# SamsungLabs/fcaf3d

Measured on AMD Instinct MI355X. Metric: scenes/sec fwd+bwd, ScanNet 100k-pt 2cm voxels, 1/2/4/8 MI355X, higher is better.
Workload: dtype f32

## Files before the change

fcaf3d_amd/csrc/norm_bn.h:

```cpp
#pragma once


__global__ void k_bn1_partial(const float* __restrict__ x, int64_t n, int C, int64_t rpb, float* __restrict__ part) {
  extern __shared__ float sm[];
  const auto [cl, rl, nrl] = lane_coord(C / 4);
  const auto [r0, r1] = row_span(rpb, n);
  const float4 sh = *reinterpret_cast<const float4*>(x + cl * 4);
  float4 a1 = make_float4(0.f, 0.f, 0.f, 0.f), a2 = a1;
  for (int64_t rb = r0 + rl; rb < r1; rb += 4 * (int64_t)nrl) {
    float4 v[4];
#pragma unroll
    for (int u = 0; u < 4; ++u) {
      const int64_t r = rb + (int64_t)u * nrl;
      v[u] = *reinterpret_cast<const float4*>(x + (r < r1 ? r : 0) * C + cl * 4);
    }
#pragma unroll
    for (int u = 0; u < 4; ++u) {
      v[u].x -= sh.x; v[u].y -= sh.y; v[u].z -= sh.z; v[u].w -= sh.w;
      a1.x += v[u].x; a1.y += v[u].y; a1.z += v[u].z; a1.w += v[u].w;
      a2.x += v[u].x * v[u].x; a2.y += v[u].y * v[u].y; a2.z += v[u].z * v[u].z; a2.w += v[u].w * v[u].w;
    }
  }
  *reinterpret_cast<float4*>(&sm[(rl * 2 + 0) * C + cl * 4]) = a1;
  *reinterpret_cast<float4*>(&sm[(rl * 2 + 1) * C + cl * 4]) = a2;
  __syncthreads();
  if (rl == 0) {
    float4 t1 = make_float4(0.f, 0.f, 0.f, 0.f), t2 = t1;
    for (int j = 0; j < nrl; ++j) {
      float4 u = *reinterpret_cast<const float4*>(&sm[(j * 2 + 0) * C + cl * 4]);
      float4 w = *reinterpret_cast<const float4*>(&sm[(j * 2 + 1) * C + cl * 4]);
      t1.x += u.x; t1.y += u.y; t1.z += u.z; t1.w += u.w;
      t2.x += w.x; t2.y += w.y; t2.z += w.z; t2.w += w.w;
    }
    float* dst = part + ((int64_t)blockIdx.x * 2) * C;
    *reinterpret_cast<float4*>(dst + cl * 4) = t1;
    *reinterpret_cast<float4*>(dst + C + cl * 4) = t2;
  }
}

__device__ static inline void bn1_reduce_parts(const float* __restrict__ part, int nb, int C, int cl, int rl, int nrl,
                                               float* sm , float4* s1, float4* s2, int CG, int c0) {
  float4 a1 = make_float4(0.f, 0.f, 0.f, 0.f), a2 = a1;
  const bool past_l1 = (int64_t)nb * C * 8 <= 32768;
  for (int b = rl; b < nb; b += nrl) {
    const float* src = part + ((int64_t)b * 2) * C + c0;
    float4 u = past_l1 ? fc_ld4(src + cl * 4) : *reinterpret_cast<const float4*>(src + cl * 4);
    float4 w = past_l1 ? fc_ld4(src + C + cl * 4) : *reinterpret_cast<const float4*>(src + C + cl * 4);
    a1.x += u.x; a1.y += u.y; a1.z += u.z; a1.w += u.w;
    a2.x += w.x; a2.y += w.y; a2.z += w.z; a2.w += w.w;
  }
  *reinterpret_cast<float4*>(&sm[(rl * 2 + 0) * CG + cl * 4]) = a1;
  *reinterpret_cast<float4*>(&sm[(rl * 2 + 1) * CG + cl * 4]) = a2;
  __syncthreads();
  float4 t1 = make_float4(0.f, 0.f, 0.f, 0.f), t2 = t1;
  for (int j = 0; j < nrl; ++j) {
    float4 u = *reinterpret_cast<const float4*>(&sm[(j * 2 + 0) * CG + cl * 4]);
    float4 w = *reinterpret_cast<const float4*>(&sm[(j * 2 + 1) * CG + cl * 4]);
    t1.x += u.x; t1.y += u.y; t1.z += u.z; t1.w += u.w;
    t2.x += w.x; t2.y += w.y; t2.z += w.z; t2.w += w.w;
  }
  *s1 = t1; *s2 = t2;
}

__global__ void k_bn1_apply(const float* __restrict__ x, int64_t n, int C, int64_t rpb, const float* __restrict__ part, int nb,
                            float eps, const float* __restrict__ gamma, const float* __restrict__ beta,
                            const float* __restrict__ residual, int act, float momentum, float* __restrict__ y,
                            float* __restrict__ mean_out, float* __restrict__ var_out, float* __restrict__ cnt_out,
                            float* __restrict__ rmean, float* __restrict__ rvar, long long* __restrict__ nbt,
                            const int* __restrict__ add_inv, const float* __restrict__ add_src) {
  extern __shared__ float sm[];
  const int c4n = C / 4;
  const int cl = threadIdx.x % c4n, rl = threadIdx.x / c4n;
  const int nrl = blockDim.x / c4n;
  float4 s1, s2;
  bn1_reduce_parts(part, nb, C, cl, rl, nrl, sm, &s1, &s2, C, 0);
  const float4 sh = *reinterpret_cast<const float4*>(x + cl * 4);
  const float inv_n = 1.f / (float)n;
  float d[4] = {s1.x * inv_n, s1.y * inv_n, s1.z * inv_n, s1.w * inv_n};
  float q[4] = {s2.x * inv_n, s2.y * inv_n, s2.z * inv_n, s2.w * inv_n};
  float shv[4] = {sh.x, sh.y, sh.z, sh.w};
  float mu[4], va[4], is[4], g[4], bt[4];
#pragma unroll
  for (int j = 0; j < 4; ++j) {
    mu[j] = shv[j] + d[j];
    va[j] = fmaxf(q[j] - d[j] * d[j], 0.f);
    is[j] = 1.f / sqrtf(va[j] + eps);
    g[j] = gamma ? gamma[cl * 4 + j] : 1.f;
    bt[j] = beta ? beta[cl * 4 + j] : 0.f;
  }
  if (blockIdx.x == 0 && rl == 0) {
    *reinterpret_cast<float4*>(mean_out + cl * 4) = make_float4(mu[0], mu[1], mu[2], mu[3]);
    *reinterpret_cast<float4*>(var_out + cl * 4) = make_float4(va[0], va[1], va[2], va[3]);
    if (cl == 0) { cnt_out[0] = (float)n; if (nbt) nbt[0] += 1; }
    if (rmean) {
#pragma unroll
      for (int j = 0; j < 4; ++j) bn_running_update(rmean, rvar, cl * 4 + j, mu[j], va[j], (float)n, momentum);
    }
  }
  const auto [r0, r1] = row_span(rpb, n);
  for (int64_t rb = r0 + rl; rb < r1; rb += 4 * (int64_t)nrl) {
    float v[4][4], rs[4][4];
#pragma unroll
    for (int u = 0; u < 4; ++u) {
      const int64_t r = rb + (int64_t)u * nrl;
      const int64_t rc = r < r1 ? r : r0;
      *reinterpret_cast<float4*>(v[u]) = *reinterpret_cast<const float4*>(x + rc * C + cl * 4);
      if (residual) *reinterpret_cast<float4*>(rs[u]) = *reinterpret_cast<const float4*>(residual + rc * C + cl * 4);
    }
#pragma unroll
    for (int u = 0; u < 4; ++u) {
      const int64_t r = rb + (int64_t)u * nrl;
      if (r >= r1) continue;
      float o[4];
#pragma unroll
      for (int j = 0; j < 4; ++j) o[j] = norm_act_elem(v[u][j], mu[j], is[j], g[j], bt[j], residual ? &rs[u][j] : nullptr, act);
      const int q = add_inv ? add_inv[r] : -1;
      if (q >= 0) {
        const float4 f = *reinterpret_cast<const float4*>(add_src + (int64_t)q * C + cl * 4);
        o[0] += f.x; o[1] += f.y; o[2] += f.z; o[3] += f.w;
      }
      *reinterpret_cast<float4*>(y + r * C + cl * 4) = *reinterpret_cast<float4*>(o);
    }
  }
}

__global__ __launch_bounds__(1024) void k_bn_finalize(const float* __restrict__ part, int nb, int C, int64_t n,
                                                      const float* __restrict__ x, float momentum, float* __restrict__ mean,
                                                      float* __restrict__ var, float* __restrict__ cnt,
                                                      float* __restrict__ rmean, float* __restrict__ rvar,
                                                      long long* __restrict__ nbt) {
  __shared__ float r1[16][65], r2[16][65];
  const int c = blockIdx.x * 64 + (threadIdx.x & 63), j = threadIdx.x >> 6;
  float a1 = 0.f, a2 = 0.f;
  if (c < C) {
    float p1[4] = {0.f, 0.f, 0.f, 0.f}, p2[4] = {0.f, 0.f, 0.f, 0.f};
    int b = j;
    for (; b + 48 < nb; b += 64) {
      float u[4], w[4];
#pragma unroll
      for (int q = 0; q < 4; ++q) {
        u[q] = fc_ld(&part[((int64_t)(b + 16 * q) * 2) * C + c]);
        w[q] = fc_ld(&part[((int64_t)(b + 16 * q) * 2 + 1) * C + c]);
      }
#pragma unroll
      for (int q = 0; q < 4; ++q) { p1[q] += u[q]; p2[q] += w[q]; }
    }
    for (; b < nb; b += 16) {
      p1[0] += fc_ld(&part[((int64_t)b * 2) * C + c]);
      p2[0] += fc_ld(&part[((int64_t)b * 2 + 1) * C + c]);
    }
    a1 = (p1[0] + p1[1]) + (p1[2] + p1[3]);
    a2 = (p2[0] + p2[1]) + (p2[2] + p2[3]);
  }
  r1[j][threadIdx.x & 63] = a1;
  r2[j][threadIdx.x & 63] = a2;
  __syncthreads();
  if (j == 0 && c < C) {
    float s1 = 0.f, s2 = 0.f;
    for (int q = 0; q < 16; ++q) { s1 += r1[q][threadIdx.x & 63]; s2 += r2[q][threadIdx.x & 63]; }
    const float inv_n = 1.f / (float)n;
    float d = s1 * inv_n;
    float mu = x[c] + d;
    float va = fmaxf(s2 * inv_n - d * d, 0.f);
    mean[c] = mu;
    var[c] = va;
    if (c == 0) { cnt[0] = (float)n; if (nbt) nbt[0] += 1; }
    if (rmean) bn_running_update(rmean, rvar, c, mu, va, (float)n, momentum);
  }
}

__global__ void k_bn1_bwd_apply(const float* __restrict__ x, const float* __restrict__ y, const float* __restrict__ gy,
                                const float* __restrict__ gy2, int64_t n, int C, int64_t rpb, const float* __restrict__ part, int nb,
                                const float* __restrict__ mean, const float* __restrict__ var, float eps,
                                const float* __restrict__ gamma, const float* __restrict__ beta, int act,
                                float* __restrict__ gx, float* __restrict__ gres, float* __restrict__ sums , int CG,
                                unsigned* __restrict__ amax_out) {
  extern __shared__ float sm[];
  const int c0 = blockIdx.y * CG;
  x += c0; gy += c0; gx += c0; mean += c0; var += c0;
  if (y) y += c0;
  if (gy2) gy2 += c0;
  if (gres) gres += c0;
  if (gamma) gamma += c0;
  if (beta) beta += c0;
  const int c4n = CG / 4;
  const int cl = threadIdx.x % c4n, rl = threadIdx.x / c4n;
  const int nrl = blockDim.x / c4n;
  float4 t1, t2;
  bn1_reduce_parts(part, nb, C, cl, rl, nrl, sm, &t1, &t2, CG, c0);
  if (blockIdx.x == 0 && rl == 0) {
    *reinterpret_cast<float4*>(sums + c0 + cl * 4) = t1;
    *reinterpret_cast<float4*>(sums + C + c0 + cl * 4) = t2;
  }
  const float inv_n = 1.f / (float)n;
  float s1[4] = {t1.x * inv_n, t1.y * inv_n, t1.z * inv_n, t1.w * inv_n};
  float s2[4] = {t2.x * inv_n, t2.y * inv_n, t2.z * inv_n, t2.w * inv_n};
  float mu[4], is[4], g[4], bt[4];
#pragma unroll
  for (int j = 0; j < 4; ++j) {
    mu[j] = mean[cl * 4 + j];
    is[j] = 1.f / sqrtf(var[cl * 4 + j] + eps);
    g[j] = gamma ? gamma[cl * 4 + j] : 1.f;
    bt[j] = beta ? beta[cl * 4 + j] : 0.f;
  }
  const bool from_y = act && y;
  const auto [r0, r1] = row_span(rpb, n);
  unsigned am = 0u;
  for (int64_t rb = r0 + rl; rb < r1; rb += 4 * (int64_t)nrl) {
    float xv[4][4], gv[4][4], yv[4][4];
#pragma unroll
    for (int u = 0; u < 4; ++u) {
      const int64_t r = rb + (int64_t)u * nrl;
      const int64_t rc = r < r1 ? r : r0;
      *reinterpret_cast<float4*>(xv[u]) = *reinterpret_cast<const float4*>(x + rc * C + cl * 4);
      *reinterpret_cast<float4*>(gv[u]) = *reinterpret_cast<const float4*>(gy + rc * C + cl * 4);
      if (gy2) {
        const float4 t2 = *reinterpret_cast<const float4*>(gy2 + rc * C + cl * 4);
        gv[u][0] += t2.x; gv[u][1] += t2.y; gv[u][2] += t2.z; gv[u][3] += t2.w;
      }
      if (from_y) *reinterpret_cast<float4*>(yv[u]) = *reinterpret_cast<const float4*>(y + rc * C + cl * 4);
    }
#pragma unroll
    for (int u = 0; u < 4; ++u) {
      const int64_t r = rb + (int64_t)u * nrl;
      if (r >= r1) continue;
      float o[4], gr[4];
#pragma unroll
      for (int j = 0; j < 4; ++j) {
        float gg = gv[u][j];
        if (from_y) gg *= act_bwd_from_y(yv[u][j], act);
        else if (act) gg *= act_bwd_from_pre(bn_pre(xv[u][j], mu[j], is[j], g[j], bt[j]), act);
        float xh = (xv[u][j] - mu[j]) * is[j];
        gr[j] = gg;
        o[j] = g[j] * is[j] * (gg - s1[j] - xh * s2[j]);
      }
      *reinterpret_cast<float4*>(gx + r * C + cl * 4) = *reinterpret_cast<float4*>(o);
      if (gres) *reinterpret_cast<float4*>(gres + r * C + cl * 4) = *reinterpret_cast<float4*>(gr);
#pragma unroll
      for (int j = 0; j < 4; ++j) amax_fold(am, o[j]);
    }
  }
  if (amax_out) amax_commit(am, amax_out);
}

__global__ void k_bn2_apply(const float* __restrict__ x, int64_t n, int C, int64_t rpb, const float* __restrict__ part, int nb, int G,
                            float eps, const float* __restrict__ gamma, const float* __restrict__ beta,
                            const float* __restrict__ residual, int act, float momentum, float* __restrict__ y,
                            float* __restrict__ mean_out, float* __restrict__ var_out, float* __restrict__ cnt_out,
                            float* __restrict__ rmean, float* __restrict__ rvar, long long* __restrict__ nbt, int CG,
                            const int* __restrict__ add_inv, const float* __restrict__ add_src, unsigned* __restrict__ amax_out) {
  extern __shared__ double smd[];
  const int c0 = blockIdx.y * CG;
  x += c0; y += c0; part += c0; mean_out += c0; var_out += c0;
  if (add_src) add_src += c0;
  if (residual) residual += c0;
  if (gamma) gamma += c0;
  if (beta) beta += c0;
  if (rmean) { rmean += c0; rvar += c0; }
  const auto [cl, rl, nrl] = lane_coord(CG / 4);
  double a1[4] = {0., 0., 0., 0.}, a2[4] = {0., 0., 0., 0.};
  const int GC = G * C;
  for (int t = rl; t < nb * G; t += nrl) {
    const int b = t / G, g = t % G;
    const float* src = part + ((int64_t)b * 2) * GC + g * C + cl * 4;
    const float4 u = fc_ld4(src), w = fc_ld4(src + GC);
    a1[0] += u.x; a1[1] += u.y; a1[2] += u.z; a1[3] += u.w;
    a2[0] += w.x; a2[1] += w.y; a2[2] += w.z; a2[3] += w.w;
  }
#pragma unroll
  for (int j = 0; j < 4; ++j) {
    smd[(rl * 2 + 0) * CG + cl * 4 + j] = a1[j];
    smd[(rl * 2 + 1) * CG + cl * 4 + j] = a2[j];
  }
  __syncthreads();
  float mu[4], va[4], is[4], g[4], bt[4];
#pragma unroll
  for (int j = 0; j < 4; ++j) {
    double t1 = 0., t2 = 0.;
    for (int q = 0; q < nrl; ++q) { t1 += smd[(q * 2 + 0) * CG + cl * 4 + j]; t2 += smd[(q * 2 + 1) * CG + cl * 4 + j]; }
    bn2_stats(t1, t2, n, &mu[j], &va[j]);
    is[j] = 1.f / sqrtf(va[j] + eps);
    g[j] = gamma ? gamma[cl * 4 + j] : 1.f;
    bt[j] = beta ? beta[cl * 4 + j] : 0.f;
  }
  if (blockIdx.x == 0 && rl == 0) {
    *reinterpret_cast<float4*>(mean_out + cl * 4) = make_float4(mu[0], mu[1], mu[2], mu[3]);
    *reinterpret_cast<float4*>(var_out + cl * 4) = make_float4(va[0], va[1], va[2], va[3]);
    if (cl == 0 && blockIdx.y == 0) { cnt_out[0] = (float)n; if (nbt) nbt[0] += 1; }
    if (rmean) {
#pragma unroll
      for (int j = 0; j < 4; ++j) bn_running_update(rmean, rvar, cl * 4 + j, mu[j], va[j], (float)n, momentum);
    }
  }
  const auto [r0, r1] = row_span(rpb, n);
  unsigned am = 0u;
  for (int64_t rb = r0 + rl; rb < r1; rb += 4 * (int64_t)nrl) {
    float v[4][4], rs[4][4];
    int q[4];
#pragma unroll
    for (int u = 0; u < 4; ++u) {
      const int64_t r = rb + (int64_t)u * nrl;
      const int64_t rc = r < r1 ? r : r0;
      *reinterpret_cast<float4*>(v[u]) = *reinterpret_cast<const float4*>(x + rc * C + cl * 4);
      if (residual) *reinterpret_cast<float4*>(rs[u]) = *reinterpret_cast<const float4*>(residual + rc * C + cl * 4);
      q[u] = add_inv ? add_inv[rc] : -1;
    }
#pragma unroll
    for (int u = 0; u < 4; ++u) {
      const int64_t r = rb + (int64_t)u * nrl;
      if (r >= r1) continue;
      float o[4];
#pragma unroll
      for (int j = 0; j < 4; ++j) o[j] = norm_act_elem(v[u][j], mu[j], is[j], g[j], bt[j], residual ? &rs[u][j] : nullptr, act);
      if (q[u] >= 0) {
        const float4 f = *reinterpret_cast<const float4*>(add_src + (int64_t)q[u] * C + cl * 4);
        o[0] += f.x; o[1] += f.y; o[2] += f.z; o[3] += f.w;
      }
      *reinterpret_cast<float4*>(y + r * C + cl * 4) = *reinterpret_cast<float4*>(o);
#pragma unroll
      for (int j = 0; j < 4; ++j) amax_fold(am, o[j]);
    }
  }
  if (amax_out) amax_commit(am, amax_out);
}

__global__ __launch_bounds__(256) void k_bn2_finalize(const float* __restrict__ part, int nb, int C, int G, int64_t n, float momentum,
                                                       float* __restrict__ mean, float* __restrict__ var, float* __restrict__ cnt,
                                                       float* __restrict__ rmean, float* __restrict__ rvar,
                                                       long long* __restrict__ nbt) {
  __shared__ double r1[FIN_SL][FIN_CB + 1], r2[FIN_SL][FIN_CB + 1];
  const int cl = threadIdx.x & (FIN_CB - 1), j = threadIdx.x / FIN_CB;
  const int c = blockIdx.x * FIN_CB + cl;
  const int GC = G * C;
  double a1 = 0., a2 = 0.;
  if (c < C) {
    double p1[4] = {0., 0., 0., 0.}, p2[4] = {0., 0., 0., 0.};
    const int total = nb * G;
    int t = j;
    for (; t + 3 * FIN_SL < total; t += 4 * FIN_SL) {
      float u[4], w[4];
#pragma unroll
      for (int q = 0; q < 4; ++q) {
        const int tt = t + FIN_SL * q, b = tt / G, g = tt % G;
        u[q] = fc_ld(&part[((int64_t)b * 2) * GC + g * C + c]);
        w[q] = fc_ld(&part[((int64_t)b * 2 + 1) * GC + g * C + c]);
      }
#pragma unroll
      for (int q = 0; q < 4; ++q) { p1[q] += u[q]; p2[q] += w[q]; }
    }
    for (; t < total; t += FIN_SL) {
      const int b = t / G, g = t % G;
      p1[0] += fc_ld(&part[((int64_t)b * 2) * GC + g * C + c]);
      p2[0] += fc_ld(&part[((int64_t)b * 2 + 1) * GC + g * C + c]);
    }
    a1 = (p1[0] + p1[1]) + (p1[2] + p1[3]);
    a2 = (p2[0] + p2[1]) + (p2[2] + p2[3]);
  }
  r1[j][cl] = a1;
  r2[j][cl] = a2;
  __syncthreads();
  if (j == 0 && c < C) {
    double s1 = 0., s2 = 0.;
    for (int q = 0; q < FIN_SL; ++q) { s1 += r1[q][cl]; s2 += r2[q][cl]; }
    float mu, va;
    bn2_stats(s1, s2, n, &mu, &va);
    mean[c] = mu;
    var[c] = va;
    if (c == 0) { cnt[0] = (float)n; if (nbt) nbt[0] += 1; }
    if (rmean) bn_running_update(rmean, rvar, c, mu, va, (float)n, momentum);
  }
}

extern "C" __global__ void k_bn_running(const float* __restrict__ mean, const float* __restrict__ var, const float* __restrict__ cnt,
                             float momentum, int C, float* __restrict__ rmean, float* __restrict__ rvar,
                             long long* __restrict__ nbt) {
  int c = blockIdx.x * blockDim.x + threadIdx.x;
  if (c == 0 && nbt) nbt[0] += 1;
  if (c >= C) return;
  float n = cnt[0];
  float unbias = n / fmaxf(n - 1.f, 1.f);
  rmean[c] = (1.f - momentum) * rmean[c] + momentum * mean[c];
  rvar[c] = (1.f - momentum) * rvar[c] + momentum * var[c] * unbias;
}
```

Before: 542.7.

## Overlap first row-tile loads with BN partial reduction and batch partial loads

In the BN backward apply and BN2 apply kernels, the first tile of activation rows is now loaded before the cross-block partial-sum reduction, so global-memory latency overlaps the reduction. The partial-sum reduction loops are unrolled by four with a scheduling barrier, putting several loads in flight at once. BN2 also prefetches gathered add_src rows and splits the per-channel stats across lanes with shuffles when CG is 64. 256-thread launch bounds are added. The cost is more live registers from the preloaded tiles, which may reduce occupancy.

```diff
diff --git a/fcaf3d_amd/csrc/norm_bn.h b/fcaf3d_amd/csrc/norm_bn.h
--- a/fcaf3d_amd/csrc/norm_bn.h
+++ b/fcaf3d_amd/csrc/norm_bn.h
@@ -38,16 +38,28 @@
   }
 }
 
+#define AP_TB 4
+
 __device__ static inline void bn1_reduce_parts(const float* __restrict__ part, int nb, int C, int cl, int rl, int nrl,
                                                float* sm , float4* s1, float4* s2, int CG, int c0) {
   float4 a1 = make_float4(0.f, 0.f, 0.f, 0.f), a2 = a1;
   const bool past_l1 = (int64_t)nb * C * 8 <= 32768;
-  for (int b = rl; b < nb; b += nrl) {
-    const float* src = part + ((int64_t)b * 2) * C + c0;
-    float4 u = past_l1 ? fc_ld4(src + cl * 4) : *reinterpret_cast<const float4*>(src + cl * 4);
-    float4 w = past_l1 ? fc_ld4(src + C + cl * 4) : *reinterpret_cast<const float4*>(src + C + cl * 4);
-    a1.x += u.x; a1.y += u.y; a1.z += u.z; a1.w += u.w;
-    a2.x += w.x; a2.y += w.y; a2.z += w.z; a2.w += w.w;
+  for (int b0 = rl; b0 < nb; b0 += AP_TB * nrl) {
+    float4 u[AP_TB], w[AP_TB];
+#pragma unroll
+    for (int q = 0; q < AP_TB; ++q) {
+      const int b = b0 + q * nrl;
+      const float* src = part + ((int64_t)(b < nb ? b : b0) * 2) * C + c0;
+      u[q] = past_l1 ? fc_ld4(src + cl * 4) : *reinterpret_cast<const float4*>(src + cl * 4);
+      w[q] = past_l1 ? fc_ld4(src + C + cl * 4) : *reinterpret_cast<const float4*>(src + C + cl * 4);
+    }
+    __builtin_amdgcn_sched_barrier(0);
+#pragma unroll
+    for (int q = 0; q < AP_TB; ++q) {
+      if (b0 + q * nrl >= nb) continue;
+      a1.x += u[q].x; a1.y += u[q].y; a1.z += u[q].z; a1.w += u[q].w;
+      a2.x += w[q].x; a2.y += w[q].y; a2.z += w[q].z; a2.w += w[q].w;
+    }
   }
   *reinterpret_cast<float4*>(&sm[(rl * 2 + 0) * CG + cl * 4]) = a1;
   *reinterpret_cast<float4*>(&sm[(rl * 2 + 1) * CG + cl * 4]) = a2;
@@ -169,7 +181,7 @@
   }
 }
 
-__global__ void k_bn1_bwd_apply(const float* __restrict__ x, const float* __restrict__ y, const float* __restrict__ gy,
+__global__ __launch_bounds__(256) void k_bn1_bwd_apply(const float* __restrict__ x, const float* __restrict__ y, const float* __restrict__ gy,
                                 const float* __restrict__ gy2, int64_t n, int C, int64_t rpb, const float* __restrict__ part, int nb,
                                 const float* __restrict__ mean, const float* __restrict__ var, float eps,
                                 const float* __restrict__ gamma, const float* __restrict__ beta, int act,
@@ -186,6 +198,31 @@
   const int c4n = CG / 4;
   const int cl = threadIdx.x % c4n, rl = threadIdx.x / c4n;
   const int nrl = blockDim.x / c4n;
+  const bool from_y = act && y;
+  const RowSpan span = row_span(rpb, n);
+  const int64_t r0 = span.r0, r1 = span.r1;
+  float xv[4][4], gv[4][4], g2[4][4], yv[4][4];
+  const auto load_rows = [&](int64_t rb) {
+#pragma unroll
+    for (int u = 0; u < 4; ++u) {
+      const int64_t r = rb + (int64_t)u * nrl;
+      const int64_t rc = r < r1 ? r : r0;
+      *reinterpret_cast<float4*>(xv[u]) = *reinterpret_cast<const float4*>(x + rc * C + cl * 4);
+      *reinterpret_cast<float4*>(gv[u]) = *reinterpret_cast<const float4*>(gy + rc * C + cl * 4);
+      if (gy2) *reinterpret_cast<float4*>(g2[u]) = *reinterpret_cast<const float4*>(gy2 + rc * C + cl * 4);
+      if (from_y) *reinterpret_cast<float4*>(yv[u]) = *reinterpret_cast<const float4*>(y + rc * C + cl * 4);
+    }
+  };
+  int64_t rb = r0 + rl;
+  if (rb < r1) load_rows(rb);
+  float mu[4], va[4], is[4], g[4], bt[4];
+#pragma unroll
+  for (int j = 0; j < 4; ++j) {
+    mu[j] = mean[cl * 4 + j];
+    va[j] = var[cl * 4 + j];
+    g[j] = gamma ? gamma[cl * 4 + j] : 1.f;
+    bt[j] = beta ? beta[cl * 4 + j] : 0.f;
+  }
   float4 t1, t2;
   bn1_reduce_parts(part, nb, C, cl, rl, nrl, sm, &t1, &t2, CG, c0);
   if (blockIdx.x == 0 && rl == 0) {
@@ -195,30 +232,14 @@
   const float inv_n = 1.f / (float)n;
   float s1[4] = {t1.x * inv_n, t1.y * inv_n, t1.z * inv_n, t1.w * inv_n};
   float s2[4] = {t2.x * inv_n, t2.y * inv_n, t2.z * inv_n, t2.w * inv_n};
-  float mu[4], is[4], g[4], bt[4];
-#pragma unroll
-  for (int j = 0; j < 4; ++j) {
-    mu[j] = mean[cl * 4 + j];
-    is[j] = 1.f / sqrtf(var[cl * 4 + j] + eps);
-    g[j] = gamma ? gamma[cl * 4 + j] : 1.f;
-    bt[j] = beta ? beta[cl * 4 + j] : 0.f;
-  }
-  const bool from_y = act && y;
-  const auto [r0, r1] = row_span(rpb, n);
+#pragma unroll
+  for (int j = 0; j < 4; ++j) is[j] = 1.f / sqrtf(va[j] + eps);
   unsigned am = 0u;
-  for (int64_t rb = r0 + rl; rb < r1; rb += 4 * (int64_t)nrl) {
-    float xv[4][4], gv[4][4], yv[4][4];
-#pragma unroll
-    for (int u = 0; u < 4; ++u) {
-      const int64_t r = rb + (int64_t)u * nrl;
-      const int64_t rc = r < r1 ? r : r0;
-      *reinterpret_cast<float4*>(xv[u]) = *reinterpret_cast<const float4*>(x + rc * C + cl * 4);
-      *reinterpret_cast<float4*>(gv[u]) = *reinterpret_cast<const float4*>(gy + rc * C + cl * 4);
-      if (gy2) {
-        const float4 t2 = *reinterpret_cast<const float4*>(gy2 + rc * C + cl * 4);
-        gv[u][0] += t2.x; gv[u][1] += t2.y; gv[u][2] += t2.z; gv[u][3] += t2.w;
-      }
-      if (from_y) *reinterpret_cast<float4*>(yv[u]) = *reinterpret_cast<const float4*>(y + rc * C + cl * 4);
+  for (bool first = true; rb < r1; rb += 4 * (int64_t)nrl, first = false) {
+    if (!first) load_rows(rb);
+    if (gy2) {
+#pragma unroll
+      for (int u = 0; u < 4; ++u) { gv[u][0] += g2[u][0]; gv[u][1] += g2[u][1]; gv[u][2] += g2[u][2]; gv[u][3] += g2[u][3]; }
     }
 #pragma unroll
     for (int u = 0; u < 4; ++u) {
@@ -243,7 +264,7 @@
   if (amax_out) amax_commit(am, amax_out);
 }
 
-__global__ void k_bn2_apply(const float* __restrict__ x, int64_t n, int C, int64_t rpb, const float* __restrict__ part, int nb, int G,
+__global__ __launch_bounds__(256) void k_bn2_apply(const float* __restrict__ x, int64_t n, int C, int64_t rpb, const float* __restrict__ part, int nb, int G,
                             float eps, const float* __restrict__ gamma, const float* __restrict__ beta,
                             const float* __restrict__ residual, int act, float momentum, float* __restrict__ y,
                             float* __restrict__ mean_out, float* __restrict__ var_out, float* __restrict__ cnt_out,
@@ -257,31 +278,90 @@
   if (gamma) gamma += c0;
   if (beta) beta += c0;
   if (rmean) { rmean += c0; rvar += c0; }
-  const auto [cl, rl, nrl] = lane_coord(CG / 4);
+  const LaneCoord lane = lane_coord(CG / 4);
+  const RowSpan span = row_span(rpb, n);
+  const int cl = lane.cl, rl = lane.rl, nrl = lane.nrl;
+  const int64_t r0 = span.r0, r1 = span.r1;
+  float v[4][4], rs[4][4];
+  int q[4];
+  const auto load_rows = [&](int64_t rb) {
+#pragma unroll
+    for (int u = 0; u < 4; ++u) {
+      const int64_t r = rb + (int64_t)u * nrl;
+      const int64_t rc = r < r1 ? r : r0;
+      *reinterpret_cast<float4*>(v[u]) = *reinterpret_cast<const float4*>(x + rc * C + cl * 4);
+      if (residual) *reinterpret_cast<float4*>(rs[u]) = *reinterpret_cast<const float4*>(residual + rc * C + cl * 4);
+      q[u] = add_inv ? add_inv[rc] : -1;
+    }
+  };
+  float4 f[4];
+  const auto load_adds = [&](int64_t rb) {
+#pragma unroll
+    for (int u = 0; u < 4; ++u)
+      if (rb + (int64_t)u * nrl < r1 && q[u] >= 0) f[u] = *reinterpret_cast<const float4*>(add_src + (int64_t)q[u] * C + cl * 4);
+  };
+  int64_t rb = r0 + rl;
+  if (rb < r1) load_rows(rb);
+  float mu[4], va[4], is[4], g[4], bt[4];
+#pragma unroll
+  for (int j = 0; j < 4; ++j) {
+    g[j] = gamma ? gamma[cl * 4 + j] : 1.f;
+    bt[j] = beta ? beta[cl * 4 + j] : 0.f;
+  }
   double a1[4] = {0., 0., 0., 0.}, a2[4] = {0., 0., 0., 0.};
-  const int GC = G * C;
-  for (int t = rl; t < nb * G; t += nrl) {
-    const int b = t / G, g = t % G;
-    const float* src = part + ((int64_t)b * 2) * GC + g * C + cl * 4;
-    const float4 u = fc_ld4(src), w = fc_ld4(src + GC);
-    a1[0] += u.x; a1[1] += u.y; a1[2] += u.z; a1[3] += u.w;
-    a2[0] += w.x; a2[1] += w.y; a2[2] += w.z; a2[3] += w.w;
-  }
+  const int GC = G * C, T = nb * G;
+  int t0 = rl;
+  do {
+    float4 u[AP_TB], w[AP_TB];
+#pragma unroll
+    for (int p = 0; p < AP_TB; ++p) {
+      const int t = t0 + p * nrl, tc = t < T ? t : T - 1;
+      const int b = tc / G, gi = tc % G;
+      const float* src = part + ((int64_t)b * 2) * GC + gi * C + cl * 4;
+      u[p] = fc_ld4(src), w[p] = fc_ld4(src + GC);
+    }
+    __builtin_amdgcn_sched_barrier(0);
+#pragma unroll
+    for (int p = 0; p < AP_TB; ++p) {
+      const bool in = t0 + p * nrl < T;
+      const float us[4] = {u[p].x, u[p].y, u[p].z, u[p].w}, ws[4] = {w[p].x, w[p].y, w[p].z, w[p].w};
+#pragma unroll
+      for (int j = 0; j < 4; ++j) {
+        const double n1 = a1[j] + us[j], n2 = a2[j] + ws[j];
+        a1[j] = in ? n1 : a1[j];
+        a2[j] = in ? n2 : a2[j];
+      }
+    }
+    t0 += AP_TB * nrl;
+  } while (t0 < T);
+  if (add_inv && rb < r1) load_adds(rb);
 #pragma unroll
   for (int j = 0; j < 4; ++j) {
     smd[(rl * 2 + 0) * CG + cl * 4 + j] = a1[j];
     smd[(rl * 2 + 1) * CG + cl * 4 + j] = a2[j];
   }
   __syncthreads();
-  float mu[4], va[4], is[4], g[4], bt[4];
-#pragma unroll
-  for (int j = 0; j < 4; ++j) {
+  if (CG == 64 && nrl == 16) {
+    const int j = rl & 3;
     double t1 = 0., t2 = 0.;
-    for (int q = 0; q < nrl; ++q) { t1 += smd[(q * 2 + 0) * CG + cl * 4 + j]; t2 += smd[(q * 2 + 1) * CG + cl * 4 + j]; }
-    bn2_stats(t1, t2, n, &mu[j], &va[j]);
-    is[j] = 1.f / sqrtf(va[j] + eps);
-    g[j] = gamma ? gamma[cl * 4 + j] : 1.f;
-    bt[j] = beta ? beta[cl * 4 + j] : 0.f;
+    for (int p = 0; p < 16; ++p) { t1 += smd[(p * 2 + 0) * CG + cl * 4 + j]; t2 += smd[(p * 2 + 1) * CG + cl * 4 + j]; }
+    float m, v;
+    bn2_stats(t1, t2, n, &m, &v);
+    const float s = 1.f / sqrtf(v + eps);
+#pragma unroll
+    for (int k = 0; k < 4; ++k) {
+      mu[k] = __shfl(m, k * 16 + cl);
+      va[k] = __shfl(v, k * 16 + cl);
+      is[k] = __shfl(s, k * 16 + cl);
+    }
+  } else {
+#pragma unroll
+    for (int j = 0; j < 4; ++j) {
+      double t1 = 0., t2 = 0.;
+      for (int p = 0; p < nrl; ++p) { t1 += smd[(p * 2 + 0) * CG + cl * 4 + j]; t2 += smd[(p * 2 + 1) * CG + cl * 4 + j]; }
+      bn2_stats(t1, t2, n, &mu[j], &va[j]);
+      is[j] = 1.f / sqrtf(va[j] + eps);
+    }
   }
   if (blockIdx.x == 0 && rl == 0) {
     *reinterpret_cast<float4*>(mean_out + cl * 4) = make_float4(mu[0], mu[1], mu[2], mu[3]);
@@ -292,18 +372,11 @@
       for (int j = 0; j < 4; ++j) bn_running_update(rmean, rvar, cl * 4 + j, mu[j], va[j], (float)n, momentum);
     }
   }
-  const auto [r0, r1] = row_span(rpb, n);
   unsigned am = 0u;
-  for (int64_t rb = r0 + rl; rb < r1; rb += 4 * (int64_t)nrl) {
-    float v[4][4], rs[4][4];
-    int q[4];
-#pragma unroll
-    for (int u = 0; u < 4; ++u) {
-      const int64_t r = rb + (int64_t)u * nrl;
-      const int64_t rc = r < r1 ? r : r0;
-      *reinterpret_cast<float4*>(v[u]) = *reinterpret_cast<const float4*>(x + rc * C + cl * 4);
-      if (residual) *reinterpret_cast<float4*>(rs[u]) = *reinterpret_cast<const float4*>(residual + rc * C + cl * 4);
-      q[u] = add_inv ? add_inv[rc] : -1;
+  for (bool first = true; rb < r1; rb += 4 * (int64_t)nrl, first = false) {
+    if (!first) {
+      load_rows(rb);
+      if (add_inv) load_adds(rb);
     }
 #pragma unroll
     for (int u = 0; u < 4; ++u) {
@@ -312,10 +385,7 @@
       float o[4];
 #pragma unroll
       for (int j = 0; j < 4; ++j) o[j] = norm_act_elem(v[u][j], mu[j], is[j], g[j], bt[j], residual ? &rs[u][j] : nullptr, act);
-      if (q[u] >= 0) {
-        const float4 f = *reinterpret_cast<const float4*>(add_src + (int64_t)q[u] * C + cl * 4);
-        o[0] += f.x; o[1] += f.y; o[2] += f.z; o[3] += f.w;
-      }
+      if (q[u] >= 0) { o[0] += f[u].x; o[1] += f[u].y; o[2] += f[u].z; o[3] += f[u].w; }
       *reinterpret_cast<float4*>(y + r * C + cl * 4) = *reinterpret_cast<float4*>(o);
 #pragma unroll
       for (int j = 0; j < 4; ++j) amax_fold(am, o[j]);
```

After: 540.1. No clear change (-0.5%).
